# lmb-freiburg/demon

Hardware: AMD Instinct MI355X
Metric: image-pairs/s full 3-iter DeMoN forward @256x192 (higher is better)
Workload: dtype f32

## Files before the change

demon_amd/csrc/conv_row.hip:

```cpp
#include <type_traits>

#include "internal.h"
#include "wino1d_tables.h"

namespace demon {

typedef float floatx4 __attribute__((ext_vector_type(4)));
typedef float floatx2 __attribute__((ext_vector_type(2)));
typedef unsigned u32x2 __attribute__((ext_vector_type(2)));

constexpr int ROW_NT = 256, ROW_TX = 64, ROW_R = 2, ROW_PW = 136, ROW_MAXC = 32;

template <int KIND, bool CAFFE>
__global__ __launch_bounds__(ROW_NT, 2) void conv_row_kernel(RowArgs a)
{
    using K = Wino1D<KIND>;
    constexpr int NUV = K::NUV, WIN = K::WIN, TAPS = K::TAPS;
    constexpr int NG = (NUV + 3) / 4;
    extern __shared__ __attribute__((aligned(16))) float smem[];
    const int csteps = a.Cin4 >> 2;
    float *Us = smem;
    float *patch = smem + csteps * NUV * 128;
    const int tid = threadIdx.x, lane = tid & 63, l15 = lane & 15, lk = lane >> 4;
    const int wave = __builtin_amdgcn_readfirstlane(tid >> 6);
// ... 151 lines not shown
{
    if (kh != 1 || (kw != 7 && kw != 9) || sh != 1 || sw != 2 || ph != 0) return false;
    if (pw != kw / 2 && pw != (kw - 2) / 2) return false;
    return Cin >= 16 && (Cin + 3) / 4 * 4 <= ROW_MAXC && Mpad == 32 && (W & 3) == 0 && (Wo & 1) == 0 && Wo == (W + 1) / 2;
}

template <int KIND, bool CAFFE>
static bool launch_row_t(const RowArgs &a, dim3 grid, size_t lds, hipStream_t s)
{
    static PerDeviceOnce once;
    if (!once.ensure([] { return hipFuncSetAttribute(reinterpret_cast<const void *>(&conv_row_kernel<KIND, CAFFE>), hipFuncAttributeMaxDynamicSharedMemorySize, 80 * 1024) == hipSuccess; })) return false;
    hipLaunchKernelGGL((conv_row_kernel<KIND, CAFFE>), grid, dim3(ROW_NT), lds, s, a);
    return true;
}

bool launch_conv_row(RowArgs a, int taps, hipStream_t stream)
{
    a.tiles_y = (a.Ho + ROW_R - 1) / ROW_R;
    a.tiles_x = (a.Wo + ROW_TX - 1) / ROW_TX;
    const int nuv = taps + 2;
    const size_t lds = sizeof(float) * ((size_t)(a.Cin4 / 4) * nuv * 128 + (size_t)a.Cin4 * ROW_R * ROW_PW);
    const int ntiles = a.N * a.tiles_y * a.tiles_x;
    static const int tpw_env = getenv("DEMON_ROW_TPW") ? atoi(getenv("DEMON_ROW_TPW")) : 0;
    const int tpw = tpw_env > 0 ? tpw_env : 3;
    const int wgs = (ntiles + tpw - 1) / tpw;
    const dim3 grid((unsigned)(wgs < 1 ? 1 : wgs));
    const bool caffe = a.pad == taps / 2;
    if (taps == 9) return caffe ? launch_row_t<3, true>(a, grid, lds, stream) : launch_row_t<3, false>(a, grid, lds, stream);
    return caffe ? launch_row_t<2, true>(a, grid, lds, stream) : launch_row_t<2, false>(a, grid, lds, stream);
}

}
```

demon_amd/csrc/conv_wino4.hip:

```cpp
#include <algorithm>
#include <type_traits>

#include "internal.h"
#include "wino1d_tables.h"

namespace demon {

typedef float floatx4 __attribute__((ext_vector_type(4)));

namespace {
__device__ __forceinline__ int w4div(int n, unsigned magic) { return magic ? (int)__umulhi((unsigned)n, magic) : n; }
}

template <int KIND> struct Wino4Kind;
template <> struct Wino4Kind<0> { using T = Wino43; };
template <> struct Wino4Kind<1> { using T = Wino4K5S2; };

template <int KIND, bool SAMEPAD> struct Wino4Pieces;
template <bool S> struct Wino4Pieces<0, S> { static constexpr int N = 3; static constexpr int off[3] = {-1, 0, 4}, len[3] = {1, 4, 1}; };
template <> struct Wino4Pieces<1, false> { static constexpr int N = 4; static constexpr int off[4] = {-2, 0, 4, 8}, len[4] = {2, 4, 4, 1}; };
template <> struct Wino4Pieces<1, true> { static constexpr int N = 4; static constexpr int off[4] = {-1, 0, 4, 8}, len[4] = {1, 4, 4, 2}; };

template <int KIND, int AXIS, int WM, int WN, int TN, int KG, bool MASK, bool SAMEPAD, bool PERSIST>
__global__ __launch_bounds__(64 * WM * WN, 2) void wino4_kernel(Wino4Args a)
{
    using K = typename Wino4Kind<KIND>::T;
    using P = Wino4Pieces<KIND, SAMEPAD>;
    constexpr int NUV = K::NUV, WIN = K::WIN, OUT = K::OUT, STRIDE = K::STRIDE, NT = 64 * WM * WN, CKS = 4 * KG;
    constexpr int BM = 16 * WM, TCOLS = 16 * WN;
    constexpr int SLOTS = TN * TCOLS;
    constexpr int TP = SLOTS + ((SLOTS & 31) ? 0 : 16);
    constexpr int NUNIT = SLOTS * CKS;
    constexpr int UNITS = (NUNIT + NT - 1) / NT;
    constexpr int NLD = AXIS == 0 ? WIN : P::N;
    constexpr int ASZ = NUV * CKS * BM, TSZ = NUV * CKS * TP;
    constexpr int A4 = NUV * BM * KG;
// ... 298 lines not shown
    const long idx = (long)blockIdx.x * 256 + threadIdx.x;
    if (idx >= (long)Cin * Mpad) return;
    const int ci = (int)(idx / Mpad), co = (int)(idx - (long)ci * Mpad);
    float w[K::TAPS];
#pragma unroll
    for (int t = 0; t < K::TAPS; ++t) w[t] = wp[((long)t * Cin + ci) * Mpad + co];
#pragma unroll
    for (int e = 0; e < K::NUV; ++e) {
        float u = 0.0f;
#pragma unroll
        for (int t = 0; t < K::TAPS; ++t) u += K::g(e, t) * w[t];
        wu[((long)e * Cin4 + ci) * Mpad + co] = u;
    }
}

int wino4_kind(int taps, int stride) { return (taps == 3 && stride == 1) ? 0 : ((taps == 5 && stride == 2) ? 1 : -1); }
int wino4_nuv(int kind) { return kind == 0 ? 6 : 11; }

void launch_wino4_repack(float *wu, const float *wp, int kind, int Cin, int Cin4, int Mpad, hipStream_t s)
{
    const long total = (long)Cin * Mpad;
    const dim3 grid((unsigned)((total + 255) / 256));
    if (kind == 0) hipLaunchKernelGGL(wino4_repack_kernel<0>, grid, dim3(256), 0, s, wu, wp, Cin, Cin4, Mpad);
    else hipLaunchKernelGGL(wino4_repack_kernel<1>, grid, dim3(256), 0, s, wu, wp, Cin, Cin4, Mpad);
}

struct W4Shape { int wm, wn, tn, kg; };
static const W4Shape kW4Shapes[] = {{4, 1, 4, 1}, {4, 1, 2, 2}, {2, 2, 4, 1}, {2, 2, 2, 2}, {4, 2, 2, 2}, {4, 2, 4, 1}, {4, 1, 1, 4}, {2, 2, 1, 4}, {2, 2, 2, 1},
                                                   {4, 2, 3, 2}, {2, 2, 3, 2}, {4, 1, 3, 2}, {2, 2, 3, 1}, {4, 2, 3, 1}};
static_assert(sizeof(kW4Shapes) / sizeof(kW4Shapes[0]) == WINO4_VARIANTS, "one shape per variant");
int wino4_variant_bm(int v) { return 16 * kW4Shapes[v].wm; }
int wino4_variant_kg(int v) { return kW4Shapes[v].kg; }

bool wino4_variant_ok(int kind, int v)
{
    if (kind < 0 || kind > 1 || v < 0 || v >= WINO4_VARIANTS) return false;
    if (kind == 1 && (v == 1 || v == 3)) return false;
    return wino4_nuv(kind) * kW4Shapes[v].tn * 4 <= 96;
}

static size_t wino4_lds_bytes(int kind, int v)
{
    const W4Shape s = kW4Shapes[v];
    const int nuv = wino4_nuv(kind), cks = 4 * s.kg, slots = s.tn * 16 * s.wn, tp = slots + ((slots & 31) ? 0 : 16);
    return sizeof(float) * (2ul * (nuv * cks * 16 * s.wm + nuv * cks * tp) + 4ul * 64 * s.wm * s.wn);
}

bool wino4_plan_geometry(Wino4Args &a, int kind, int variant, int axis, bool flat)
{
    if (!wino4_variant_ok(kind, variant)) return false;
    const W4Shape s = kW4Shapes[variant];
    const int taps = kind == 0 ? 3 : 5, stride = kind == 0 ? 1 : 2;
    if (a.Mpad % (16 * s.wm)) return false;
    if (a.pad != taps / 2 && !(stride == 2 && a.pad == (taps - stride) / 2)) return false;
    if (axis == 1 && ((a.W & 3) || (a.Wo & 3))) return false;
    const int lines = axis == 0 ? (a.Ho + 3) / 4 : a.Ho, positions = axis == 0 ? a.Wo : a.Wo / 4;
    const int blockw = 16 * s.wn;
    int subl = 1;
    if (positions < blockw) {
        if (positions < 2 || (positions & (positions - 1))) return false;
        subl = blockw / positions;
        if (subl > 16) return false;
    }
    a.sub_shift = subl == 1 ? 0 : (subl == 2 ? 1 : (subl == 4 ? 2 : (subl == 8 ? 3 : 4)));
    a.pb_shift = 0;
    while ((1 << a.pb_shift) < blockw / subl) ++a.pb_shift;
    auto magic = [](int d) { return d <= 1 ? 0u : (unsigned)((0x100000000ull + (unsigned)d - 1) / (unsigned)d); };
// ... 29 lines not shown
template <int KIND, int AXIS, int WM, int WN, int TN, int KG, bool MASK, bool SAMEPAD, bool PERSIST>
static bool launch_w4m(const Wino4Args &a, dim3 grid, size_t lds, hipStream_t s)
{
    static PerDeviceOnce once;
    if (lds > 48 * 1024 &&
        !once.ensure([] { return hipFuncSetAttribute(reinterpret_cast<const void *>(&wino4_kernel<KIND, AXIS, WM, WN, TN, KG, MASK, SAMEPAD, PERSIST>), hipFuncAttributeMaxDynamicSharedMemorySize, 160 * 1024) == hipSuccess; }))
        return false;
    hipLaunchKernelGGL((wino4_kernel<KIND, AXIS, WM, WN, TN, KG, MASK, SAMEPAD, PERSIST>), grid, dim3(64 * WM * WN), lds, s, a);
    return true;
}

template <int KIND, int AXIS, int WM, int WN, int TN, int KG>
static bool launch_w4(const Wino4Args &a, dim3 grid, size_t lds, hipStream_t s, bool persist)
{
    using K = typename Wino4Kind<KIND>::T;
    if constexpr (K::NUV * TN * 4 <= 96 && !(KIND == 1 && TN == 2 && KG == 2 && WM * WN == 4)) {
        const bool mask = a.Cin % (4 * KG) != 0;
        const bool same = KIND == 1 && AXIS == 1 && a.pad != K::TAPS / 2;
        if constexpr (KIND == 1 && AXIS == 1) {
            if (same) {
                if (persist) return false;
                return mask ? launch_w4m<KIND, AXIS, WM, WN, TN, KG, true, true, false>(a, grid, lds, s) : launch_w4m<KIND, AXIS, WM, WN, TN, KG, false, true, false>(a, grid, lds, s);
            }
        }
        if (persist) {
            if constexpr (KIND == 0 && (TN <= 2 || (TN == 3 && KG == 1))) {
                if (!mask) return launch_w4m<KIND, AXIS, WM, WN, TN, KG, false, false, true>(a, grid, lds, s);
            }
            return false;
        }
        return mask ? launch_w4m<KIND, AXIS, WM, WN, TN, KG, true, false, false>(a, grid, lds, s) : launch_w4m<KIND, AXIS, WM, WN, TN, KG, false, false, false>(a, grid, lds, s);
    }
    return false;
}
// ... 4 lines not shown
    switch (variant) {
        case 0: return launch_w4<KIND, AXIS, 4, 1, 4, 1>(a, grid, lds, s, persist);
        case 1: return launch_w4<KIND, AXIS, 4, 1, 2, 2>(a, grid, lds, s, persist);
        case 2: return launch_w4<KIND, AXIS, 2, 2, 4, 1>(a, grid, lds, s, persist);
        case 3: return launch_w4<KIND, AXIS, 2, 2, 2, 2>(a, grid, lds, s, persist);
        case 4: return launch_w4<KIND, AXIS, 4, 2, 2, 2>(a, grid, lds, s, persist);
        case 5: return launch_w4<KIND, AXIS, 4, 2, 4, 1>(a, grid, lds, s, persist);
        case 6: return launch_w4<KIND, AXIS, 4, 1, 1, 4>(a, grid, lds, s, persist);
        case 7: return launch_w4<KIND, AXIS, 2, 2, 1, 4>(a, grid, lds, s, persist);
        case 8: return launch_w4<KIND, AXIS, 2, 2, 2, 1>(a, grid, lds, s, persist);
        case 9: return launch_w4<KIND, AXIS, 4, 2, 3, 2>(a, grid, lds, s, persist);
        case 10: return launch_w4<KIND, AXIS, 2, 2, 3, 2>(a, grid, lds, s, persist);
        case 11: return launch_w4<KIND, AXIS, 4, 1, 3, 2>(a, grid, lds, s, persist);
        case 12: return launch_w4<KIND, AXIS, 2, 2, 3, 1>(a, grid, lds, s, persist);
        case 13: return launch_w4<KIND, AXIS, 4, 2, 3, 1>(a, grid, lds, s, persist);
        default: return false;
    }
}

int wino4_persist_grid(const Wino4Args &a, int kind, int variant)
{
    if (!wino4_variant_ok(kind, variant)) return 0;
    if (kind != 0 || !(kW4Shapes[variant].tn <= 2 || (kW4Shapes[variant].tn == 3 && kW4Shapes[variant].kg == 1))) return 0;
    static int cus = [] { hipDeviceProp_t p; int d = 0; return (hipGetDevice(&d) == hipSuccess && hipGetDeviceProperties(&p, d) == hipSuccess && p.multiProcessorCount > 0) ? p.multiProcessorCount : 256; }();
    const W4Shape sh = kW4Shapes[variant];
    const long tiles = wino4_workgroups(a, variant);
    const int by_waves = 8 / (sh.wm * sh.wn), by_lds = (int)(160 * 1024 / wino4_lds_bytes(kind, variant));
    const long slots = (long)(g_active_cus > 0 ? g_active_cus : cus) * std::max(1, std::min(by_waves, by_lds));
    if (tiles <= slots) return 0;
    const long per = (tiles + slots - 1) / slots;
    long grid = (tiles + per - 1) / per;
    grid = (grid + 7) / 8 * 8;
    return (int)std::min(grid, tiles);
}

bool launch_wino4(const Wino4Args &a_in, int kind, int variant, int axis, hipStream_t stream, bool persist)
{
    const int bm = wino4_variant_bm(variant);
    Wino4Args a = a_in;
    if (persist && a.flat) return false;
    a.gx = (a.flat ? 1 : a.N) * a.rows_y * a.cols_x;
    a.gy = (a.Cout + bm - 1) / bm;
    a.m_gx = a.gx <= 1 ? 0u : (unsigned)((0x100000000ull + (unsigned)a.gx - 1) / (unsigned)a.gx);
    dim3 grid((unsigned)a.gx, (unsigned)a.gy, 1);
    if (persist) {
        const int g = wino4_persist_grid(a, kind, variant);
        if (g <= 0) return false;
        grid = dim3((unsigned)g, 1, 1);
    }
    const size_t lds = wino4_lds_bytes(kind, variant);
    if (kind == 0) return axis == 0 ? launch_w4_variant<0, 0>(a, variant, grid, lds, stream, persist) : launch_w4_variant<0, 1>(a, variant, grid, lds, stream, persist);
    if (kind == 1) return axis == 0 ? launch_w4_variant<1, 0>(a, variant, grid, lds, stream, persist) : launch_w4_variant<1, 1>(a, variant, grid, lds, stream, persist);
    return false;
}

}
```

demon_amd/csrc/demon_api.hip:

```cpp
#include <hip/hip_runtime.h>
#include <dlfcn.h>
#include <rccl/rccl.h>
#include <stdio.h>
#include <stdlib.h>
#include <string.h>

#include <algorithm>
#include <cmath>
#include <array>
#include <chrono>
#include <functional>
#include <mutex>
#include <map>
#include <memory>
#include <string>
#include <vector>

#include "../../include/demon_hip.h"
#include "internal.h"

using namespace demon;

namespace {

// ... 878 lines not shown
    t.N = a.N; t.Cin = L->Cin; t.H = a.H; t.W = a.W; t.in_n_stride = a.in_n_stride;
    t.Cout = L->Cout; t.Mpad = L->Mpad; t.Ho = a.Ho; t.Wo = a.Wo; t.out_n_stride = a.out_n_stride; t.out_plane = a.out_plane;
    t.pad = L->ph; t.act = a.act; t.xcd = a.xcd; t.tiles_y = t.tiles_x = 0;
    launch_conv_thin(t, s);
    snprintf(g_kernel_tag, sizeof g_kernel_tag, "conv_thin<32x512,t%d>", L->kh);
    g_last_kernel = g_kernel_tag;
    return true;
}

bool row_applies(const Layer *L)
{
    return L->kind == Layer::CONV && !L->scale && L->d_w1 != nullptr && L->wino1d_cross() == 1 &&
           conv_row_shape_ok(L->kh, L->kw, L->sh, L->sw, L->ph, L->pw, L->Cin, L->Mpad, L->in.W, L->out.W);
}

bool run_row(const Layer *L, const ConvArgs &a, hipStream_t s)
{
    refresh_stream_weights(L, s);
    RowArgs r;
    r.in = a.in; r.out = a.out; r.wu = L->d_w1; r.bias = a.bias;
    r.N = a.N; r.Cin = L->Cin; r.Cin4 = L->Cin4(); r.H = a.H; r.W = a.W; r.in_n_stride = a.in_n_stride;
    r.Cout = L->Cout; r.Ho = a.Ho; r.Wo = a.Wo; r.out_n_stride = a.out_n_stride; r.out_plane = a.out_plane;
    r.pad = L->pw; r.act = a.act; r.tiles_y = r.tiles_x = 0;
    if (!launch_conv_row(r, L->kw, s)) return false;
    snprintf(g_kernel_tag, sizeof g_kernel_tag, "conv_row<32x128,t%d>", L->kw);
    g_last_kernel = g_kernel_tag;
    return true;
}

void run_mfma(const ConvArgs &a_in, ConvPlan plan, int ncls, hipStream_t s)
{
    launch_conv_mfma(a_in, plan, ncls, s);
    snprintf(g_kernel_tag, sizeof g_kernel_tag, "conv_mfma<%dx%d>%s", conv_tile_bm(plan.tile), conv_tile_bn(plan.tile), split_suffix(plan.ksplit));
    g_last_kernel = g_kernel_tag;
}

template <class Clamp>
void run_bf16(const Layer *L, ConvArgs a, long P, float *ws, hipStream_t s, Clamp clamp_split)
{
// ... 34 lines not shown
                    run_stream(L, a, tile, clamp_split(ks), s);
                    return;
                }
            } else if (kind == 5) {
                if (L->stream_ok() && tile >= 0 && tile < FRAG_VARIANTS && L->Mpad % frag_variant_bm(tile) == 0) {
                    run_frag(L, a, tile, clamp_split(ks), s);
                    return;
                }
            } else if (kind == 10) {
                if (wino1d_applies(L) && run_wino1d(L, a, tile, clamp_split(ks % 1000), s)) return;
            } else if (kind == 15) {
                if (run_wino3(L, a, tile, s)) return;
            } else if (kind == 16) {
                if (run_wino4(L, a, tile, s, ks)) return;
            } else if (kind == 13) {
                if (row_applies(L) && run_row(L, a, s)) return;
            } else if (kind == 12) {
                if (thin_applies(L) && run_thin(L, a, s)) return;
            } else if (kind == 11) {
                if (dense_stream_applies(L) && run_dense_stream(L, a, tile, clamp_split(ks % 1000), s)) return;
            } else if (kind == 8) {
                if (wino_applies(L) && tile >= 0 && tile < WINO_VARIANTS && run_wino(L, a, tile, clamp_split(ks % 1000), s)) return;
            } else if (kind == 1) {
                PatchPlan pp;
                if (tile >= 0 && tile < PTILE_COUNT && plan_patch(L, n, ws, pp, tile, ks / 1000 - 1)) {
                    if (ks % 1000 > 0) pp.a.ksplit = ks % 1000 < pp.a.nsteps_total ? ks % 1000 : pp.a.nsteps_total;
                    launch_patch_plan(L, pp, a, P, ws, s);
                    return;
                }
            } else if (tile >= 0 && tile < TILE_COUNT && L->Mpad % conv_tile_bm(tile) == 0) {
                run_mfma(a, ConvPlan{tile, clamp_split(ks < 1 ? 1 : std::min(ks % 1000, L->Kpad / 16))}, L->ncls, s);
// ... 8 lines not shown
            if (t.kind == 3 && small_applies(L)) {
                run_small(L, a, s);
                return;
            }
            if ((t.kind == 4 || t.kind == 7) && L->stream_ok() && L->Mpad % stream_variant_bm(t.tile) == 0) {
                run_stream(L, a, t.tile, t.kind == 7 ? 1 : clamp_split(t.ksplit), s);
                return;
            }
            if ((t.kind == 5 || t.kind == 6) && L->stream_ok() && L->Mpad % frag_variant_bm(t.tile) == 0) {
                run_frag(L, a, t.tile, t.kind == 6 ? 1 : clamp_split(t.ksplit), s);
                return;
            }
            if (t.kind == 8 && wino_applies(L) && run_wino(L, a, t.tile, clamp_split(t.ksplit), s)) return;
            if (t.kind == 10 && wino1d_applies(L) && run_wino1d(L, a, t.tile, clamp_split(t.ksplit), s)) return;
            if (t.kind == 12 && thin_applies(L) && run_thin(L, a, s)) return;
            if (t.kind == 13 && row_applies(L) && run_row(L, a, s)) return;
            if (t.kind == 15 && run_wino3(L, a, t.tile, s)) return;
            if (t.kind == 16 && run_wino4(L, a, t.tile, s, t.ksplit)) return;
            if (t.kind == 11 && dense_stream_applies(L) && run_dense_stream(L, a, t.tile, clamp_split(t.ksplit), s)) return;
            if (t.kind == 1) {
                PatchPlan pp;
                const int tw = t.ksplit / 1000 - 1, ks = t.ksplit % 1000;
                if (plan_patch(L, n, ws, pp, t.tile, tw)) {
                    if (ks > 0) pp.a.ksplit = ks < pp.a.nsteps_total ? ks : pp.a.nsteps_total;
                    launch_patch_plan(L, pp, a, P, ws, s);
                    return;
                }
            } else if (t.kind == 0) {
                run_mfma(a, ConvPlan{t.tile, clamp_split(t.ksplit)}, L->ncls, s);
                return;
            }
// ... 145 lines not shown
        }
    }
    if (wino1d_applies(L)) {
        for (int v = 0; v < WINO1D_VARIANTS; ++v) {
            Wino1Args w;
            if (!fill_wino1d_args(L, a, v, w)) continue;
            const int nsteps = w.csteps * wino1d_variant_kg(v);
            const long wgs = wino1d_workgroups(w, v);
            for (int ks : {1, 2, 3, 4, 6, 8}) {
                if (ks > 1 && (ks > nsteps / 8 || wgs * ks > 4096 || (long)ks * L->Mpad * P > kSplitKWorkspaceFloats)) continue;
                if (wgs * ks < 64) continue;
                cands.push_back({10, v, ks});
            }
        }
    }
    if (wino4_applies(L)) {
        for (int v = 0; v < WINO4_VARIANTS; ++v) {
            Wino4Args w;
            if (fill_wino4_args(L, a, v, w) && wino4_workgroups(w, v) >= 128) {
                cands.push_back({16, v, 1});
                w.gx = (int)wino4_workgroups(w, v); w.gy = 1;
                if (L->Cin % (4 * wino4_variant_kg(v)) == 0 && wino4_persist_grid(w, L->wino4_kind_of(), v) > 0) cands.push_back({16, v, 2});
            }
            if (fill_wino4_args(L, a, v, w, true) && wino4_workgroups(w, v) >= 96) cands.push_back({16, v, 3});
        }
    }
    if (wino3_applies(L)) {
        for (int v = 0; v < WINO3_VARIANTS; ++v) {
            Wino3Args w;
            if (fill_wino3_args(L, a, v, w) && wino3_workgroups(w, v) >= 128) cands.push_back({15, v, 1});
        }
    }
    if (thin_applies(L)) cands.push_back({12, 0, 1});
    if (row_applies(L)) cands.push_back({13, 0, 1});
    if (dense_stream_applies(L)) {
        const long blocks = (long)(L->Mpad / 128) * ((n + 31) / 32);
        for (int ks : {1, 2, 3, 4, 6, 8, 9, 12, 16, 18, 24, 32, 36, 48, 64}) {
            if (!dense_stream_geometry_ok(L->Cin, L->Mpad, ks)) continue;
            if (ks > 1 && ((long)ks * L->Mpad * P > kSplitKWorkspaceFloats || blocks * ks > 4096)) continue;
            if (blocks * ks < 64 && ks < 64) continue;
            for (int v = 0; v < DENSE_VARIANTS; ++v) cands.push_back({11, v, ks});
        }
    }
    if (wino_applies(L) && !getenv("DEMON_NO_WINO")) {
        const int nsteps = (L->Cin + 3) / 4;
        for (int v = 0; v < WINO_VARIANTS; ++v) {
            WinoArgs w;
            w.N = n; w.H = a.H; w.W = a.W; w.Mpad = L->Mpad; w.Cin = L->Cin; w.nsteps_total = nsteps;
            if (!wino_plan_geometry(w, v, n)) continue;
// ... 1255 lines not shown

int demon_plan_set(demon_ctx *c, int n, const char *layer_name, int kind, int tile, int ksplit)
{
    if (!c || !layer_name || n < 1 || n > c->max_batch) return fail(c, DEMON_ERR_INVALID, "bad argument");
    if (kind < 0 || kind > 16 || kind == 2 || kind == 9 || tile < 0 ||
        tile >= (kind == 16 ? (int)WINO4_VARIANTS : kind == 15 ? (int)WINO3_VARIANTS : kind >= 12 ? 1 : kind == 11 ? (int)DENSE_VARIANTS : kind == 10 ? (int)WINO1D_VARIANTS : kind == 8 ? (int)WINO_VARIANTS : (kind == 1 ? (int)PTILE_COUNT : ((kind == 4 || kind == 7) ? (int)STREAM_VARIANTS : ((kind == 5 || kind == 6) ? (int)FRAG_VARIANTS : (int)TILE_COUNT)))) || ksplit < 0)
        return fail(c, DEMON_ERR_INVALID, "bad plan entry");
    if (kind != 1 && ksplit >= 1000)
        return fail(c, DEMON_ERR_INVALID, "ksplit >= 1000 is only meaningful for the patch-staged kernel (pixel-tile shape)");
    for (auto &L : c->layers)
        if (L->name == layer_name) {
            if (kind == 0 && L->Mpad % conv_tile_bm(tile)) return fail(c, DEMON_ERR_INVALID, "tile does not divide Cout");
            if (kind == 3 && !small_applies(L.get())) return fail(c, DEMON_ERR_INVALID, "the small-Cout kernel does not apply to this layer");
            if (kind == 8 && !wino_applies(L.get())) return fail(c, DEMON_ERR_INVALID, "the minimal-filtering kernel applies to transposed convs only");
            if (kind == 10 && !wino1d_applies(L.get())) return fail(c, DEMON_ERR_INVALID, "no 1-D minimal-filtering form for this layer");
            if (kind == 16 && !wino4_applies(L.get())) return fail(c, DEMON_ERR_INVALID, "conv_wino4.hip applies to k x 1 / 1 x k convs with 3 taps stride 1 or 5 taps stride 2 and >= 16 input channels only");
            if (kind == 15 && !wino3_applies(L.get())) return fail(c, DEMON_ERR_INVALID, "conv_wino3.hip applies to 3 x 3 convs with >= 16 input channels, stride 1 (rows of even length) or stride 2 (rows of a multiple of 8 pixels, >= 64)");
            if (kind == 13 && !row_applies(L.get())) return fail(c, DEMON_ERR_INVALID, "conv_row.hip applies to 1 x 7 / 1 x 9 stride-2 convs with at most 32 channels on both sides only");
            if (kind == 12 && !thin_applies(L.get())) return fail(c, DEMON_ERR_INVALID, "conv_thin.hip applies to the 9 x 1 stride-2 first layer (Cin <= 6, Cout <= 32) only");
            if (kind == 11 && !dense_stream_applies(L.get())) return fail(c, DEMON_ERR_INVALID, "the weight-streaming kernel applies to dense layers only");
            if (kind == 4 && (!L->stream_ok() || L->Mpad % stream_variant_bm(tile))) return fail(c, DEMON_ERR_INVALID, "the streaming kernel does not apply to this layer");
            if (kind == 5 && (!L->stream_ok() || L->Mpad % frag_variant_bm(tile))) return fail(c, DEMON_ERR_INVALID, "the fragment-tiled kernel does not apply to this layer");
            if (kind == 6 || kind == 7) {
                bool ok = false;
                for (auto &pr : c->chain_pairs) ok = ok || (pr.first == L.get() && chain_shape_ok(pr.first, pr.second, kind, tile));
                if (!ok) return fail(c, DEMON_ERR_INVALID, "this layer cannot run chained with a 1 x k partner on that variant");
            }
            for (auto &g : c->graphs) hipGraphExecDestroy(g.second);
            c->graphs.clear();
            L->tuned[n] = Layer::Tuned{kind, tile, (kind == 0 || kind == 4 || kind == 5) && ksplit < 1 ? 1 : ksplit};
            return DEMON_OK;
// ... 1049 lines not shown
```

demon_amd/csrc/internal.h:

```cpp
#pragma once
#include <hip/hip_runtime.h>
#include <stdint.h>

#include <atomic>
#include <string>
#include <vector>

namespace demon {

struct PerDeviceOnce {
    std::atomic<unsigned long long> done{0};
    template <class F>
    bool ensure(F &&configure)
    {
        int dev = 0;
        if (hipGetDevice(&dev) != hipSuccess || dev < 0 || dev > 63) return configure();
        if (done.load(std::memory_order_acquire) >> dev & 1ull) return true;
        if (!configure()) return false;
        done.fetch_or(1ull << dev, std::memory_order_release);
        return true;
    }
};

struct View {
// ... 294 lines not shown
    int N, Cin, Cin4, H, W, Ho, Wo;
    long in_n_stride;
    int Cout, Mpad;
    long out_n_stride, out_plane;
    int act, pad, csteps;
    int rows_y, cols_x;
    int sub_shift, pb_shift;
    int xcd;
    unsigned m_colsx, m_rowsy;
    int gx, gy;
    unsigned m_gx;
    int flat, lines_img, nlines;
    unsigned m_lines;
    int in_img_bytes, out_img_bytes;
};
constexpr int WINO4_VARIANTS = 14;
int wino4_kind(int taps, int stride);
int wino4_nuv(int kind);
int wino4_variant_bm(int v);
int wino4_variant_kg(int v);
bool wino4_variant_ok(int kind, int v);
bool wino4_plan_geometry(Wino4Args &a, int kind, int variant, int axis, bool flat = false);
long wino4_workgroups(const Wino4Args &a, int variant);
void launch_wino4_repack(float *wu, const float *wp, int kind, int Cin, int Cin4, int Mpad, hipStream_t s);
int wino4_persist_grid(const Wino4Args &a, int kind, int variant);
bool launch_wino4(const Wino4Args &a, int kind, int variant, int axis, hipStream_t stream, bool persist = false);

struct DenseArgs {
    const float *x;
    float *out;
    const float *wd;
    const float *bias;
    float *ws;
    int N, K, Cout, Mpad;
    long x_n_stride, out_n_stride;
    int act, ksplit;
// ... 20 lines not shown
void launch_conv_thin(ThinArgs a, hipStream_t stream);

struct RowArgs {
    const float *in;
    float *out;
    const float *wu;
    const float *bias;
    int N, Cin, Cin4, H, W;
    long in_n_stride;
    int Cout, Ho, Wo;
    long out_n_stride, out_plane;
    int pad, act;
    int tiles_y, tiles_x;
};
bool conv_row_shape_ok(int kh, int kw, int sh, int sw, int ph, int pw, int Cin, int Mpad, int W, int Wo);
bool launch_conv_row(RowArgs a, int taps, hipStream_t stream);

struct SmallConvArgs {
    const float *in;
    float *out;
    const float *wp;
    const float *bias;
    const float *scale;
    int Cin, Cout, Mpad, H, W, act;
    long in_n_stride, out_n_stride;
};
bool conv_small_applies(int kh, int kw, int sh, int sw, int Cin, int Cout);
void launch_conv_small(const SmallConvArgs &a, int N, hipStream_t s);
void launch_motion_tail(const float *x, const float *w2, const float *b2, const float *w3, const float *b3, float *motion,
                        float *rot, float *trans, float *scale, int N, int K2, int M2pad, int M3pad, hipStream_t s);

// ... 67 lines not shown
```

demon_amd/csrc/wino1d_tables.h:

```cpp
#pragma once

namespace demon {

template <int KIND> struct Wino1D;

template <> struct Wino1D<0> {
    static constexpr int TAPS = 3, STRIDE = 1, NUV = 4, WIN = 4;
    static __host__ __device__ __forceinline__ float g(int e, int t) {
        constexpr float G[NUV][TAPS] = {{-1.0f, 0.0f, 0.0f}, {1.0f, 1.0f, 1.0f}, {1.0f, -1.0f, 1.0f}, {0.0f, 0.0f, 1.0f}};
        return G[e][t];
    }
    static __device__ __forceinline__ void input(const float (&d)[WIN], float (&t)[NUV]) {
    t[0] = -d[0] + d[2];
    { const float s = d[2], a = d[1]; t[1] = s + a; t[2] = s - a; }
    t[3] = -d[1] + d[3];
    }
    template <class T> static __device__ __forceinline__ void output(const T (&m)[NUV], T &o0, T &o1) {
        o0 = m[0] + (1.0f / 2.0f) * m[1] + (1.0f / 2.0f) * m[2];
        o1 = (1.0f / 2.0f) * m[1] - (1.0f / 2.0f) * m[2] + m[3];
    }
};

template <> struct Wino1D<1> {
    static constexpr int TAPS = 5, STRIDE = 2, NUV = 7, WIN = 7;
// ... 118 lines not shown
    t[3] = -d[2] + d[6];
    t[4] = 2.0f * d[2] - d[4] - 2.0f * d[6] + d[8];
    t[5] = d[1];
    t[6] = d[3];
    t[7] = d[5];
    t[8] = d[7];
    }
    template <class T> static __device__ __forceinline__ void output(const T (&m)[NUV], T (&o)[OUT]) {
        o[0] = (1.0f / 2.0f) * m[0] + (1.0f / 2.0f) * m[1] + (1.0f / 6.0f) * m[2] + (1.0f / 6.0f) * m[3] + m[5];
        o[1] = (1.0f / 2.0f) * m[1] - (1.0f / 6.0f) * m[2] + (1.0f / 3.0f) * m[3] + m[6];
        o[2] = (1.0f / 2.0f) * m[1] + (1.0f / 6.0f) * m[2] + (2.0f / 3.0f) * m[3] + m[7];
        o[3] = (1.0f / 2.0f) * m[1] - (1.0f / 6.0f) * m[2] + (4.0f / 3.0f) * m[3] + m[4] + m[8];
    }
};

}
```

demon_amd/kernel_names.py:

```python
import functools
import os
import re

CSRC = os.path.join(os.path.dirname(os.path.abspath(__file__)), "csrc")


@functools.lru_cache(None)
def frag_variants():
    src = open(os.path.join(CSRC, "conv_frag.hip")).read()
    table = {}
    for m in re.finditer(r"case (\d+): launch_frag_instance<([\d, ]+)>", src):
        table[int(m.group(1))] = tuple(int(x) for x in m.group(2).split(","))
    m = re.search(r"default: launch_frag_instance<([\d, ]+)>", src)
    if m:
        table[max(table) + 1] = tuple(int(x) for x in m.group(1).split(","))
    return table


def kernel_tag(name):
    m = re.search(r"conv_mfma_kernel<(\d+), (\d+)", name)
    if m:
        return "conv_mfma<%sx%s>" % m.groups()
    m = re.search(r"conv_bf16_kernel<(\d+), (\d+)", name)
    if m:
# ... 43 lines not shown
    if m:
        shape = tuple(map(int, m.groups()[:4]))
        form = int(m.group(6))
        if form == 2:
            shapes2 = {(4, 1, 2, 1): 16, (2, 2, 2, 1): 17, (4, 2, 2, 1): 18, (8, 1, 2, 1): 19}
            return "wino3rows<s2t3x3,v%d>" % shapes2.get(shape, -1)
        if form == 1:
            shapes4 = {(2, 2, 2, 2): 8, (4, 1, 2, 2): 9, (2, 2, 3, 1): 10, (4, 1, 3, 1): 11, (1, 4, 2, 1): 12, (1, 4, 3, 1): 13, (2, 1, 2, 2): 14, (4, 2, 3, 1): 15}
            return "wino3rows<f4t3x3,v%d>" % shapes4.get(shape, -1)
        shapes3 = {(2, 2, 4, 1): 0, (2, 4, 4, 1): 1, (4, 1, 4, 1): 2, (4, 2, 4, 1): 3, (1, 4, 4, 1): 4, (1, 4, 2, 2): 5, (2, 2, 2, 2): 6, (4, 1, 2, 2): 7}
        return "wino3rows<t3x3,v%d>" % shapes3.get(shape, -1)
    m = re.search(r"wino4_kernel<(\d+), (\d+), (\d+), (\d+), (\d+), (\d+), (true|false), (true|false), (true|false)", name)
    if m:
        kind, axis, wm, wn, tn, kg = map(int, m.groups()[:6])
        shapes4 = {(4, 1, 4, 1): 0, (4, 1, 2, 2): 1, (2, 2, 4, 1): 2, (2, 2, 2, 2): 3, (4, 2, 2, 2): 4, (4, 2, 4, 1): 5, (4, 1, 1, 4): 6, (2, 2, 1, 4): 7, (2, 2, 2, 1): 8,
                   (4, 2, 3, 2): 9, (2, 2, 3, 2): 10, (4, 1, 3, 2): 11, (2, 2, 3, 1): 12, (4, 2, 3, 1): 13}
        return "wino4<t%d,v%d%s>" % (3 if kind == 0 else 5, shapes4.get((wm, wn, tn, kg), -1), ",walk" if m.group(9) == "true" else "")
    m = re.search(r"conv_row_kernel<(\d+), ", name)
    if m:
        return "conv_row<32x128,t%d>" % (3 + 2 * int(m.group(1)))
    m = re.search(r"conv_thin_kernel<(\d+)", name)
    if m:
        return "conv_thin<32x512,t%s>" % m.group(1)
    m = re.search(r"dense_stream_kernel<(true|false)", name)
    if m:
        return "dense_stream<128x32,v%d>" % (1 if m.group(1) == "true" else 0)
    m = re.search(r"deconv4_kernel<(\d+), (\d+), (\d+)", name)
    if m:
        bm, wm, wn = map(int, m.groups())
        return "deconv4<%dx%d>" % (bm, wn * 32)
    m = re.search(r"demon::(\w+?)_kernel", name)
    return m.group(1) if m else name.split("(")[0]
# ... 43 lines not shown
```

Before: 4660.

## Add Winograd F(4) kernels for 7- and 9-tap stride-2 convs and row-conv grid options

Adds 1-D Winograd transform tables for 7- and 9-tap stride-2 filters and instantiates the wino4 kernel for them, with two new tile shapes and per-axis validity rules. It also lets the row-conv launcher take tiles-per-workgroup from the tuner (6, 12, or a whole-launch grid sized to twice the CU count). Both kinds of candidate are only enumerated when the tuner runs with more than one lane. The goal is to cut multiply work on the large-kernel stride-2 layers and to reduce workgroup overhead in the row kernel. The higher-tap Winograd transforms carry larger constants, which risks float32 accuracy loss, and they add compile time.

```diff
diff --git a/demon_amd/csrc/conv_row.hip b/demon_amd/csrc/conv_row.hip
--- a/demon_amd/csrc/conv_row.hip
+++ b/demon_amd/csrc/conv_row.hip
@@ -1,3 +1,4 @@
+#include <algorithm>
 #include <type_traits>
 
 #include "internal.h"
@@ -189,16 +190,19 @@
     return true;
 }
 
-bool launch_conv_row(RowArgs a, int taps, hipStream_t stream)
+bool launch_conv_row(RowArgs a, int taps, hipStream_t stream, int tpw_plan)
 {
     a.tiles_y = (a.Ho + ROW_R - 1) / ROW_R;
     a.tiles_x = (a.Wo + ROW_TX - 1) / ROW_TX;
     const int nuv = taps + 2;
     const size_t lds = sizeof(float) * ((size_t)(a.Cin4 / 4) * nuv * 128 + (size_t)a.Cin4 * ROW_R * ROW_PW);
     const int ntiles = a.N * a.tiles_y * a.tiles_x;
-    static const int tpw_env = getenv("DEMON_ROW_TPW") ? atoi(getenv("DEMON_ROW_TPW")) : 0;
-    const int tpw = tpw_env > 0 ? tpw_env : 3;
-    const int wgs = (ntiles + tpw - 1) / tpw;
+    const int tpw = (tpw_plan == 6 || tpw_plan == 12 || tpw_plan == kRowWholeLaunch) ? tpw_plan : 3;
+    int wgs = (ntiles + tpw - 1) / tpw;
+    if (tpw_plan == kRowWholeLaunch) {
+        static int cus = [] { hipDeviceProp_t p; int d = 0; return (hipGetDevice(&d) == hipSuccess && hipGetDeviceProperties(&p, d) == hipSuccess && p.multiProcessorCount > 0) ? p.multiProcessorCount : 256; }();
+        wgs = std::min(ntiles, 2 * (g_active_cus > 0 ? g_active_cus : cus));
+    }
     const dim3 grid((unsigned)(wgs < 1 ? 1 : wgs));
     const bool caffe = a.pad == taps / 2;
     if (taps == 9) return caffe ? launch_row_t<3, true>(a, grid, lds, stream) : launch_row_t<3, false>(a, grid, lds, stream);
diff --git a/demon_amd/csrc/conv_wino4.hip b/demon_amd/csrc/conv_wino4.hip
--- a/demon_amd/csrc/conv_wino4.hip
+++ b/demon_amd/csrc/conv_wino4.hip
@@ -15,11 +15,17 @@
 template <int KIND> struct Wino4Kind;
 template <> struct Wino4Kind<0> { using T = Wino43; };
 template <> struct Wino4Kind<1> { using T = Wino4K5S2; };
+template <> struct Wino4Kind<2> { using T = Wino4K7S2; };
+template <> struct Wino4Kind<3> { using T = Wino4K9S2; };
 
 template <int KIND, bool SAMEPAD> struct Wino4Pieces;
 template <bool S> struct Wino4Pieces<0, S> { static constexpr int N = 3; static constexpr int off[3] = {-1, 0, 4}, len[3] = {1, 4, 1}; };
 template <> struct Wino4Pieces<1, false> { static constexpr int N = 4; static constexpr int off[4] = {-2, 0, 4, 8}, len[4] = {2, 4, 4, 1}; };
 template <> struct Wino4Pieces<1, true> { static constexpr int N = 4; static constexpr int off[4] = {-1, 0, 4, 8}, len[4] = {1, 4, 4, 2}; };
+template <> struct Wino4Pieces<2, false> { static constexpr int N = 5; static constexpr int off[5] = {-3, -2, 0, 4, 8}, len[5] = {1, 2, 4, 4, 2}; };
+template <> struct Wino4Pieces<2, true> { static constexpr int N = 5; static constexpr int off[5] = {-2, 0, 4, 8, 10}, len[5] = {2, 4, 4, 2, 1}; };
+template <> struct Wino4Pieces<3, false> { static constexpr int N = 5; static constexpr int off[5] = {-4, 0, 4, 8, 10}, len[5] = {4, 4, 4, 2, 1}; };
+template <> struct Wino4Pieces<3, true> { static constexpr int N = 5; static constexpr int off[5] = {-3, -2, 0, 4, 8}, len[5] = {1, 2, 4, 4, 4}; };
 
 template <int KIND, int AXIS, int WM, int WN, int TN, int KG, bool MASK, bool SAMEPAD, bool PERSIST>
 __global__ __launch_bounds__(64 * WM * WN, 2) void wino4_kernel(Wino4Args a)
@@ -348,29 +354,50 @@
     }
 }
 
-int wino4_kind(int taps, int stride) { return (taps == 3 && stride == 1) ? 0 : ((taps == 5 && stride == 2) ? 1 : -1); }
-int wino4_nuv(int kind) { return kind == 0 ? 6 : 11; }
+int wino4_kind(int taps, int stride)
+{
+    if (taps == 3 && stride == 1) return 0;
+    if (stride != 2) return -1;
+    return taps == 5 ? 1 : (taps == 7 ? 2 : (taps == 9 ? 3 : -1));
+}
+int wino4_nuv(int kind) { return kind == 0 ? 6 : (kind == 1 ? 11 : (kind == 2 ? 13 : 15)); }
+static int wino4_taps(int kind) { return kind == 0 ? 3 : 2 * kind + 3; }
 
 void launch_wino4_repack(float *wu, const float *wp, int kind, int Cin, int Cin4, int Mpad, hipStream_t s)
 {
     const long total = (long)Cin * Mpad;
     const dim3 grid((unsigned)((total + 255) / 256));
     if (kind == 0) hipLaunchKernelGGL(wino4_repack_kernel<0>, grid, dim3(256), 0, s, wu, wp, Cin, Cin4, Mpad);
-    else hipLaunchKernelGGL(wino4_repack_kernel<1>, grid, dim3(256), 0, s, wu, wp, Cin, Cin4, Mpad);
+    else if (kind == 1) hipLaunchKernelGGL(wino4_repack_kernel<1>, grid, dim3(256), 0, s, wu, wp, Cin, Cin4, Mpad);
+    else if (kind == 2) hipLaunchKernelGGL(wino4_repack_kernel<2>, grid, dim3(256), 0, s, wu, wp, Cin, Cin4, Mpad);
+    else hipLaunchKernelGGL(wino4_repack_kernel<3>, grid, dim3(256), 0, s, wu, wp, Cin, Cin4, Mpad);
 }
 
 struct W4Shape { int wm, wn, tn, kg; };
 static const W4Shape kW4Shapes[] = {{4, 1, 4, 1}, {4, 1, 2, 2}, {2, 2, 4, 1}, {2, 2, 2, 2}, {4, 2, 2, 2}, {4, 2, 4, 1}, {4, 1, 1, 4}, {2, 2, 1, 4}, {2, 2, 2, 1},
-                                                   {4, 2, 3, 2}, {2, 2, 3, 2}, {4, 1, 3, 2}, {2, 2, 3, 1}, {4, 2, 3, 1}};
+                                                   {4, 2, 3, 2}, {2, 2, 3, 2}, {4, 1, 3, 2}, {2, 2, 3, 1}, {4, 2, 3, 1},
+                                                   {2, 2, 1, 2}, {4, 2, 1, 2}};
 static_assert(sizeof(kW4Shapes) / sizeof(kW4Shapes[0]) == WINO4_VARIANTS, "one shape per variant");
 int wino4_variant_bm(int v) { return 16 * kW4Shapes[v].wm; }
 int wino4_variant_kg(int v) { return kW4Shapes[v].kg; }
 
-bool wino4_variant_ok(int kind, int v)
-{
-    if (kind < 0 || kind > 1 || v < 0 || v >= WINO4_VARIANTS) return false;
-    if (kind == 1 && (v == 1 || v == 3)) return false;
-    return wino4_nuv(kind) * kW4Shapes[v].tn * 4 <= 96;
+constexpr bool w4_shape_built(int kind, int axis, int wm, int wn, int tn, int kg)
+{
+    if (kind <= 1) {
+        if (tn == 1 && kg == 2) return false;
+        if (kind == 1 && tn == 2 && kg == 2 && wm * wn == 4) return false;
+        return (kind == 0 ? 6 : 11) * tn * 4 <= 96;
+    }
+    if (tn == 1 && kg == 2) return true;
+    if (kind == 2) return (tn == 2 && kg == 1 && wm == 2 && wn == 2) || (axis == 1 && tn == 1 && kg == 4);
+    return axis == 1 && tn == 1 && kg == 4 && wm == 2 && wn == 2;
+}
+
+bool wino4_variant_ok(int kind, int v, int axis)
+{
+    if (kind < 0 || kind > 3 || v < 0 || v >= WINO4_VARIANTS) return false;
+    const W4Shape s = kW4Shapes[v];
+    return w4_shape_built(kind, axis, s.wm, s.wn, s.tn, s.kg);
 }
 
 static size_t wino4_lds_bytes(int kind, int v)
@@ -382,9 +409,9 @@
 
 bool wino4_plan_geometry(Wino4Args &a, int kind, int variant, int axis, bool flat)
 {
-    if (!wino4_variant_ok(kind, variant)) return false;
+    if (!wino4_variant_ok(kind, variant, axis)) return false;
     const W4Shape s = kW4Shapes[variant];
-    const int taps = kind == 0 ? 3 : 5, stride = kind == 0 ? 1 : 2;
+    const int taps = wino4_taps(kind), stride = kind == 0 ? 1 : 2;
     if (a.Mpad % (16 * s.wm)) return false;
     if (a.pad != taps / 2 && !(stride == 2 && a.pad == (taps - stride) / 2)) return false;
     if (axis == 1 && ((a.W & 3) || (a.Wo & 3))) return false;
@@ -444,10 +471,10 @@
 static bool launch_w4(const Wino4Args &a, dim3 grid, size_t lds, hipStream_t s, bool persist)
 {
     using K = typename Wino4Kind<KIND>::T;
-    if constexpr (K::NUV * TN * 4 <= 96 && !(KIND == 1 && TN == 2 && KG == 2 && WM * WN == 4)) {
+    if constexpr (w4_shape_built(KIND, AXIS, WM, WN, TN, KG)) {
         const bool mask = a.Cin % (4 * KG) != 0;
-        const bool same = KIND == 1 && AXIS == 1 && a.pad != K::TAPS / 2;
-        if constexpr (KIND == 1 && AXIS == 1) {
+        const bool same = KIND >= 1 && AXIS == 1 && a.pad != K::TAPS / 2;
+        if constexpr (KIND >= 1 && AXIS == 1) {
             if (same) {
                 if (persist) return false;
                 return mask ? launch_w4m<KIND, AXIS, WM, WN, TN, KG, true, true, false>(a, grid, lds, s) : launch_w4m<KIND, AXIS, WM, WN, TN, KG, false, true, false>(a, grid, lds, s);
@@ -482,14 +509,16 @@
         case 11: return launch_w4<KIND, AXIS, 4, 1, 3, 2>(a, grid, lds, s, persist);
         case 12: return launch_w4<KIND, AXIS, 2, 2, 3, 1>(a, grid, lds, s, persist);
         case 13: return launch_w4<KIND, AXIS, 4, 2, 3, 1>(a, grid, lds, s, persist);
+        case 14: return launch_w4<KIND, AXIS, 2, 2, 1, 2>(a, grid, lds, s, persist);
+        case 15: return launch_w4<KIND, AXIS, 4, 2, 1, 2>(a, grid, lds, s, persist);
         default: return false;
     }
 }
 
 int wino4_persist_grid(const Wino4Args &a, int kind, int variant)
 {
-    if (!wino4_variant_ok(kind, variant)) return 0;
-    if (kind != 0 || !(kW4Shapes[variant].tn <= 2 || (kW4Shapes[variant].tn == 3 && kW4Shapes[variant].kg == 1))) return 0;
+    if (kind != 0 || !wino4_variant_ok(kind, variant, 0)) return 0;
+    if (!(kW4Shapes[variant].tn <= 2 || (kW4Shapes[variant].tn == 3 && kW4Shapes[variant].kg == 1))) return 0;
     static int cus = [] { hipDeviceProp_t p; int d = 0; return (hipGetDevice(&d) == hipSuccess && hipGetDeviceProperties(&p, d) == hipSuccess && p.multiProcessorCount > 0) ? p.multiProcessorCount : 256; }();
     const W4Shape sh = kW4Shapes[variant];
     const long tiles = wino4_workgroups(a, variant);
@@ -519,6 +548,8 @@
     const size_t lds = wino4_lds_bytes(kind, variant);
     if (kind == 0) return axis == 0 ? launch_w4_variant<0, 0>(a, variant, grid, lds, stream, persist) : launch_w4_variant<0, 1>(a, variant, grid, lds, stream, persist);
     if (kind == 1) return axis == 0 ? launch_w4_variant<1, 0>(a, variant, grid, lds, stream, persist) : launch_w4_variant<1, 1>(a, variant, grid, lds, stream, persist);
+    if (kind == 2) return axis == 0 ? launch_w4_variant<2, 0>(a, variant, grid, lds, stream, persist) : launch_w4_variant<2, 1>(a, variant, grid, lds, stream, persist);
+    if (kind == 3) return axis == 0 ? launch_w4_variant<3, 0>(a, variant, grid, lds, stream, persist) : launch_w4_variant<3, 1>(a, variant, grid, lds, stream, persist);
     return false;
 }
 
diff --git a/demon_amd/csrc/demon_api.hip b/demon_amd/csrc/demon_api.hip
--- a/demon_amd/csrc/demon_api.hip
+++ b/demon_amd/csrc/demon_api.hip
@@ -916,7 +916,7 @@
            conv_row_shape_ok(L->kh, L->kw, L->sh, L->sw, L->ph, L->pw, L->Cin, L->Mpad, L->in.W, L->out.W);
 }
 
-bool run_row(const Layer *L, const ConvArgs &a, hipStream_t s)
+bool run_row(const Layer *L, const ConvArgs &a, hipStream_t s, int tpw = 0)
 {
     refresh_stream_weights(L, s);
     RowArgs r;
@@ -924,7 +924,7 @@
     r.N = a.N; r.Cin = L->Cin; r.Cin4 = L->Cin4(); r.H = a.H; r.W = a.W; r.in_n_stride = a.in_n_stride;
     r.Cout = L->Cout; r.Ho = a.Ho; r.Wo = a.Wo; r.out_n_stride = a.out_n_stride; r.out_plane = a.out_plane;
     r.pad = L->pw; r.act = a.act; r.tiles_y = r.tiles_x = 0;
-    if (!launch_conv_row(r, L->kw, s)) return false;
+    if (!launch_conv_row(r, L->kw, s, tpw)) return false;
     snprintf(g_kernel_tag, sizeof g_kernel_tag, "conv_row<32x128,t%d>", L->kw);
     g_last_kernel = g_kernel_tag;
     return true;
@@ -989,7 +989,7 @@
             } else if (kind == 16) {
                 if (run_wino4(L, a, tile, s, ks)) return;
             } else if (kind == 13) {
-                if (row_applies(L) && run_row(L, a, s)) return;
+                if (row_applies(L) && run_row(L, a, s, ks)) return;
             } else if (kind == 12) {
                 if (thin_applies(L) && run_thin(L, a, s)) return;
             } else if (kind == 11) {
@@ -1028,7 +1028,7 @@
             if (t.kind == 8 && wino_applies(L) && run_wino(L, a, t.tile, clamp_split(t.ksplit), s)) return;
             if (t.kind == 10 && wino1d_applies(L) && run_wino1d(L, a, t.tile, clamp_split(t.ksplit), s)) return;
             if (t.kind == 12 && thin_applies(L) && run_thin(L, a, s)) return;
-            if (t.kind == 13 && row_applies(L) && run_row(L, a, s)) return;
+            if (t.kind == 13 && row_applies(L) && run_row(L, a, s, t.ksplit)) return;
             if (t.kind == 15 && run_wino3(L, a, t.tile, s)) return;
             if (t.kind == 16 && run_wino4(L, a, t.tile, s, t.ksplit)) return;
             if (t.kind == 11 && dense_stream_applies(L) && run_dense_stream(L, a, t.tile, clamp_split(t.ksplit), s)) return;
@@ -1204,7 +1204,7 @@
             }
         }
     }
-    if (wino4_applies(L)) {
+    if (wino4_applies(L) && (L->wino4_kind_of() <= 1 || c->opt_tune_lanes > 1)) {
         for (int v = 0; v < WINO4_VARIANTS; ++v) {
             Wino4Args w;
             if (fill_wino4_args(L, a, v, w) && wino4_workgroups(w, v) >= 128) {
@@ -1222,7 +1222,10 @@
         }
     }
     if (thin_applies(L)) cands.push_back({12, 0, 1});
-    if (row_applies(L)) cands.push_back({13, 0, 1});
+    if (row_applies(L)) {
+        cands.push_back({13, 0, 1});
+        if (c->opt_tune_lanes > 1) for (int tpw : {6, 12, kRowWholeLaunch}) cands.push_back({13, 0, tpw});
+    }
     if (dense_stream_applies(L)) {
         const long blocks = (long)(L->Mpad / 128) * ((n + 31) / 32);
         for (int ks : {1, 2, 3, 4, 6, 8, 9, 12, 16, 18, 24, 32, 36, 48, 64}) {
@@ -2508,7 +2511,7 @@
             if (kind == 3 && !small_applies(L.get())) return fail(c, DEMON_ERR_INVALID, "the small-Cout kernel does not apply to this layer");
             if (kind == 8 && !wino_applies(L.get())) return fail(c, DEMON_ERR_INVALID, "the minimal-filtering kernel applies to transposed convs only");
             if (kind == 10 && !wino1d_applies(L.get())) return fail(c, DEMON_ERR_INVALID, "no 1-D minimal-filtering form for this layer");
-            if (kind == 16 && !wino4_applies(L.get())) return fail(c, DEMON_ERR_INVALID, "conv_wino4.hip applies to k x 1 / 1 x k convs with 3 taps stride 1 or 5 taps stride 2 and >= 16 input channels only");
+            if (kind == 16 && !wino4_applies(L.get())) return fail(c, DEMON_ERR_INVALID, "conv_wino4.hip applies to k x 1 / 1 x k convs with 3 taps stride 1 or 5 / 7 / 9 taps stride 2 and >= 16 input channels only");
             if (kind == 15 && !wino3_applies(L.get())) return fail(c, DEMON_ERR_INVALID, "conv_wino3.hip applies to 3 x 3 convs with >= 16 input channels, stride 1 (rows of even length) or stride 2 (rows of a multiple of 8 pixels, >= 64)");
             if (kind == 13 && !row_applies(L.get())) return fail(c, DEMON_ERR_INVALID, "conv_row.hip applies to 1 x 7 / 1 x 9 stride-2 convs with at most 32 channels on both sides only");
             if (kind == 12 && !thin_applies(L.get())) return fail(c, DEMON_ERR_INVALID, "conv_thin.hip applies to the 9 x 1 stride-2 first layer (Cin <= 6, Cout <= 32) only");
diff --git a/demon_amd/csrc/internal.h b/demon_amd/csrc/internal.h
--- a/demon_amd/csrc/internal.h
+++ b/demon_amd/csrc/internal.h
@@ -332,12 +332,12 @@
     unsigned m_lines;
     int in_img_bytes, out_img_bytes;
 };
-constexpr int WINO4_VARIANTS = 14;
+constexpr int WINO4_VARIANTS = 16;
 int wino4_kind(int taps, int stride);
 int wino4_nuv(int kind);
 int wino4_variant_bm(int v);
 int wino4_variant_kg(int v);
-bool wino4_variant_ok(int kind, int v);
+bool wino4_variant_ok(int kind, int v, int axis);
 bool wino4_plan_geometry(Wino4Args &a, int kind, int variant, int axis, bool flat = false);
 long wino4_workgroups(const Wino4Args &a, int variant);
 void launch_wino4_repack(float *wu, const float *wp, int kind, int Cin, int Cin4, int Mpad, hipStream_t s);
@@ -388,7 +388,8 @@
     int tiles_y, tiles_x;
 };
 bool conv_row_shape_ok(int kh, int kw, int sh, int sw, int ph, int pw, int Cin, int Mpad, int W, int Wo);
-bool launch_conv_row(RowArgs a, int taps, hipStream_t stream);
+constexpr int kRowWholeLaunch = 1000;
+bool launch_conv_row(RowArgs a, int taps, hipStream_t stream, int tiles_per_workgroup = 0);
 
 struct SmallConvArgs {
     const float *in;
diff --git a/demon_amd/csrc/wino1d_tables.h b/demon_amd/csrc/wino1d_tables.h
--- a/demon_amd/csrc/wino1d_tables.h
+++ b/demon_amd/csrc/wino1d_tables.h
@@ -156,4 +156,59 @@
     }
 };
 
+struct Wino4K7S2 {
+    static constexpr int TAPS = 7, STRIDE = 2, NUV = 13, WIN = 13, OUT = 4;
+    static __host__ __device__ __forceinline__ float g(int e, int t) {
+        constexpr float G[NUV][TAPS] = {{-1.0f, 0.0f, 0.0f, 0.0f, 0.0f, 0.0f, 0.0f}, {-1.0f, 0.0f, -1.0f, 0.0f, -1.0f, 0.0f, -1.0f}, {1.0f, 0.0f, -1.0f, 0.0f, 1.0f, 0.0f, -1.0f}, {1.0f, 0.0f, 2.0f, 0.0f, 4.0f, 0.0f, 8.0f}, {-1.0f, 0.0f, 2.0f, 0.0f, -4.0f, 0.0f, 8.0f}, {8.0f, 0.0f, 4.0f, 0.0f, 2.0f, 0.0f, 1.0f}, {0.0f, 0.0f, 0.0f, 0.0f, 0.0f, 0.0f, 1.0f}, {0.0f, 1.0f, 0.0f, 0.0f, 0.0f, 0.0f, 0.0f}, {0.0f, -1.0f, 0.0f, -1.0f, 0.0f, -1.0f, 0.0f}, {0.0f, -1.0f, 0.0f, 1.0f, 0.0f, -1.0f, 0.0f}, {0.0f, 1.0f, 0.0f, 2.0f, 0.0f, 4.0f, 0.0f}, {0.0f, 1.0f, 0.0f, -2.0f, 0.0f, 4.0f, 0.0f}, {0.0f, 0.0f, 0.0f, 0.0f, 0.0f, 1.0f, 0.0f}};
+        return G[e][t];
+    }
+    static __device__ __forceinline__ void input(const float (&d)[WIN], float (&t)[NUV]) {
+    t[0] = -4.0f * d[0] + 8.0f * d[2] + 5.0f * d[4] - 10.0f * d[6] - d[8] + 2.0f * d[10];
+    t[1] = 4.0f * d[2] - 4.0f * d[4] - 9.0f * d[6] + d[8] + 2.0f * d[10];
+    t[2] = -4.0f * d[2] + 12.0f * d[4] - 7.0f * d[6] - 3.0f * d[8] + 2.0f * d[10];
+    t[3] = 2.0f * d[2] - 3.0f * d[4] - 4.0f * d[6] + 3.0f * d[8] + 2.0f * d[10];
+    t[4] = -2.0f * d[2] + 5.0f * d[4] - 5.0f * d[8] + 2.0f * d[10];
+    t[5] = 4.0f * d[2] - 5.0f * d[6] + d[10];
+    t[6] = -4.0f * d[2] + 8.0f * d[4] + 5.0f * d[6] - 10.0f * d[8] - d[10] + 2.0f * d[12];
+    t[7] = 4.0f * d[1] - 5.0f * d[5] + d[9];
+    { const float s = -4.0f * d[5] + d[9], a = -4.0f * d[3] + d[7]; t[8] = s + a; t[9] = s - a; }
+    { const float s = -d[5] + d[9], a = -2.0f * d[3] + 2.0f * d[7]; t[10] = s + a; t[11] = s - a; }
+    t[12] = 4.0f * d[3] - 5.0f * d[7] + d[11];
+    }
+    template <class T> static __device__ __forceinline__ void output(const T (&m)[NUV], T (&o)[OUT]) {
+        o[0] = (1.0f / 4.0f) * m[0] + (1.0f / 6.0f) * m[1] + (1.0f / 18.0f) * m[2] + (1.0f / 72.0f) * m[3] + (1.0f / 120.0f) * m[4] + (4.0f / 45.0f) * m[5] + (1.0f / 4.0f) * m[7] + (1.0f / 6.0f) * m[8] + (1.0f / 6.0f) * m[9] + (1.0f / 24.0f) * m[10] + (1.0f / 24.0f) * m[11];
+        o[1] = (1.0f / 6.0f) * m[1] - (1.0f / 18.0f) * m[2] + (1.0f / 36.0f) * m[3] - (1.0f / 60.0f) * m[4] + (2.0f / 45.0f) * m[5] + (1.0f / 6.0f) * m[8] - (1.0f / 6.0f) * m[9] + (1.0f / 12.0f) * m[10] - (1.0f / 12.0f) * m[11];
+        o[2] = (1.0f / 6.0f) * m[1] + (1.0f / 18.0f) * m[2] + (1.0f / 18.0f) * m[3] + (1.0f / 30.0f) * m[4] + (1.0f / 45.0f) * m[5] + (1.0f / 6.0f) * m[8] + (1.0f / 6.0f) * m[9] + (1.0f / 6.0f) * m[10] + (1.0f / 6.0f) * m[11];
+        o[3] = (1.0f / 6.0f) * m[1] - (1.0f / 18.0f) * m[2] + (1.0f / 9.0f) * m[3] - (1.0f / 15.0f) * m[4] + (1.0f / 90.0f) * m[5] + (1.0f / 2.0f) * m[6] + (1.0f / 6.0f) * m[8] - (1.0f / 6.0f) * m[9] + (1.0f / 3.0f) * m[10] - (1.0f / 3.0f) * m[11] + m[12];
+    }
+};
+
+struct Wino4K9S2 {
+    static constexpr int TAPS = 9, STRIDE = 2, NUV = 15, WIN = 15, OUT = 4;
+    static __host__ __device__ __forceinline__ float g(int e, int t) {
+        constexpr float G[NUV][TAPS] = {{-1.0f, 0.0f, 0.0f, 0.0f, 0.0f, 0.0f, 0.0f, 0.0f, 0.0f}, {-1.0f, 0.0f, -1.0f, 0.0f, -1.0f, 0.0f, -1.0f, 0.0f, -1.0f}, {-1.0f, 0.0f, 1.0f, 0.0f, -1.0f, 0.0f, 1.0f, 0.0f, -1.0f}, {1.0f, 0.0f, 2.0f, 0.0f, 4.0f, 0.0f, 8.0f, 0.0f, 16.0f}, {1.0f, 0.0f, -2.0f, 0.0f, 4.0f, 0.0f, -8.0f, 0.0f, 16.0f}, {16.0f, 0.0f, 8.0f, 0.0f, 4.0f, 0.0f, 2.0f, 0.0f, 1.0f}, {16.0f, 0.0f, -8.0f, 0.0f, 4.0f, 0.0f, -2.0f, 0.0f, 1.0f}, {0.0f, 0.0f, 0.0f, 0.0f, 0.0f, 0.0f, 0.0f, 0.0f, 1.0f}, {0.0f, -1.0f, 0.0f, 0.0f, 0.0f, 0.0f, 0.0f, 0.0f, 0.0f}, {0.0f, -1.0f, 0.0f, -1.0f, 0.0f, -1.0f, 0.0f, -1.0f, 0.0f}, {0.0f, 1.0f, 0.0f, -1.0f, 0.0f, 1.0f, 0.0f, -1.0f, 0.0f}, {0.0f, 1.0f, 0.0f, 2.0f, 0.0f, 4.0f, 0.0f, 8.0f, 0.0f}, {0.0f, -1.0f, 0.0f, 2.0f, 0.0f, -4.0f, 0.0f, 8.0f, 0.0f}, {0.0f, 8.0f, 0.0f, 4.0f, 0.0f, 2.0f, 0.0f, 1.0f, 0.0f}, {0.0f, 0.0f, 0.0f, 0.0f, 0.0f, 0.0f, 0.0f, 1.0f, 0.0f}};
+        return G[e][t];
+    }
+    static __device__ __forceinline__ void input(const float (&d)[WIN], float (&t)[NUV]) {
+    t[0] = -4.0f * d[0] + 21.0f * d[4] - 21.0f * d[8] + 4.0f * d[12];
+    { const float s = 4.0f * d[4] - 17.0f * d[8] + 4.0f * d[12], a = 4.0f * d[2] - 17.0f * d[6] + 4.0f * d[10]; t[1] = s + a; t[2] = s - a; }
+    { const float s = d[4] - 5.0f * d[8] + 4.0f * d[12], a = 2.0f * d[2] - 10.0f * d[6] + 8.0f * d[10]; t[3] = s + a; t[4] = s - a; }
+    { const float s = 8.0f * d[4] - 10.0f * d[8] + 2.0f * d[12], a = 4.0f * d[2] - 5.0f * d[6] + d[10]; t[5] = s + a; t[6] = s - a; }
+    t[7] = -4.0f * d[2] + 21.0f * d[6] - 21.0f * d[10] + 4.0f * d[14];
+    t[8] = -4.0f * d[1] + 8.0f * d[3] + 5.0f * d[5] - 10.0f * d[7] - d[9] + 2.0f * d[11];
+    t[9] = 4.0f * d[3] - 4.0f * d[5] - 9.0f * d[7] + d[9] + 2.0f * d[11];
+    t[10] = -4.0f * d[3] + 12.0f * d[5] - 7.0f * d[7] - 3.0f * d[9] + 2.0f * d[11];
+    t[11] = 2.0f * d[3] - 3.0f * d[5] - 4.0f * d[7] + 3.0f * d[9] + 2.0f * d[11];
+    t[12] = -2.0f * d[3] + 5.0f * d[5] - 5.0f * d[9] + 2.0f * d[11];
+    t[13] = 4.0f * d[3] - 5.0f * d[7] + d[11];
+    t[14] = -4.0f * d[3] + 8.0f * d[5] + 5.0f * d[7] - 10.0f * d[9] - d[11] + 2.0f * d[13];
+    }
+    template <class T> static __device__ __forceinline__ void output(const T (&m)[NUV], T (&o)[OUT]) {
+        o[0] = (1.0f / 4.0f) * m[0] + (1.0f / 18.0f) * m[1] + (1.0f / 18.0f) * m[2] + (1.0f / 360.0f) * m[3] + (1.0f / 360.0f) * m[4] + (1.0f / 45.0f) * m[5] + (1.0f / 45.0f) * m[6] + (1.0f / 4.0f) * m[8] + (1.0f / 6.0f) * m[9] + (1.0f / 18.0f) * m[10] + (1.0f / 72.0f) * m[11] + (1.0f / 120.0f) * m[12] + (4.0f / 45.0f) * m[13];
+        o[1] = (1.0f / 18.0f) * m[1] - (1.0f / 18.0f) * m[2] + (1.0f / 180.0f) * m[3] - (1.0f / 180.0f) * m[4] + (1.0f / 90.0f) * m[5] - (1.0f / 90.0f) * m[6] + (1.0f / 6.0f) * m[9] - (1.0f / 18.0f) * m[10] + (1.0f / 36.0f) * m[11] - (1.0f / 60.0f) * m[12] + (2.0f / 45.0f) * m[13];
+        o[2] = (1.0f / 18.0f) * m[1] + (1.0f / 18.0f) * m[2] + (1.0f / 90.0f) * m[3] + (1.0f / 90.0f) * m[4] + (1.0f / 180.0f) * m[5] + (1.0f / 180.0f) * m[6] + (1.0f / 6.0f) * m[9] + (1.0f / 18.0f) * m[10] + (1.0f / 18.0f) * m[11] + (1.0f / 30.0f) * m[12] + (1.0f / 45.0f) * m[13];
+        o[3] = (1.0f / 18.0f) * m[1] - (1.0f / 18.0f) * m[2] + (1.0f / 45.0f) * m[3] - (1.0f / 45.0f) * m[4] + (1.0f / 360.0f) * m[5] - (1.0f / 360.0f) * m[6] + (1.0f / 4.0f) * m[7] + (1.0f / 6.0f) * m[9] - (1.0f / 18.0f) * m[10] + (1.0f / 9.0f) * m[11] - (1.0f / 15.0f) * m[12] + (1.0f / 90.0f) * m[13] + (1.0f / 2.0f) * m[14];
+    }
+};
+
 }
diff --git a/demon_amd/kernel_names.py b/demon_amd/kernel_names.py
--- a/demon_amd/kernel_names.py
+++ b/demon_amd/kernel_names.py
@@ -81,8 +81,8 @@
     if m:
         kind, axis, wm, wn, tn, kg = map(int, m.groups()[:6])
         shapes4 = {(4, 1, 4, 1): 0, (4, 1, 2, 2): 1, (2, 2, 4, 1): 2, (2, 2, 2, 2): 3, (4, 2, 2, 2): 4, (4, 2, 4, 1): 5, (4, 1, 1, 4): 6, (2, 2, 1, 4): 7, (2, 2, 2, 1): 8,
-                   (4, 2, 3, 2): 9, (2, 2, 3, 2): 10, (4, 1, 3, 2): 11, (2, 2, 3, 1): 12, (4, 2, 3, 1): 13}
-        return "wino4<t%d,v%d%s>" % (3 if kind == 0 else 5, shapes4.get((wm, wn, tn, kg), -1), ",walk" if m.group(9) == "true" else "")
+                   (4, 2, 3, 2): 9, (2, 2, 3, 2): 10, (4, 1, 3, 2): 11, (2, 2, 3, 1): 12, (4, 2, 3, 1): 13, (2, 2, 1, 2): 14, (4, 2, 1, 2): 15}
+        return "wino4<t%d,v%d%s>" % (3 if kind == 0 else 3 + 2 * kind, shapes4.get((wm, wn, tn, kg), -1), ",walk" if m.group(9) == "true" else "")
     m = re.search(r"conv_row_kernel<(\d+), ", name)
     if m:
         return "conv_row<32x128,t%d>" % (3 + 2 * int(m.group(1)))
```

New measurement: 4748, median of 6. +1.9%, better.
